# a-rtemis99/hpc_suffix_array

Measured on AMD Instinct MI355X. Metric: suffixes sorted/sec + ms/doubling-round, 1 GiB input at 1/2/4/8 MI355X, higher is better.
Workload: dtype u32

## Files before the change

hpc_suffix_array_amd/_native.py:

```python
from __future__ import annotations

import ctypes
import os
import subprocess

PKG_DIR = os.path.dirname(os.path.abspath(__file__))
LIB_PATH = os.path.join(PKG_DIR, "lib", "libsa_hip.so")
LIB_PATH = os.environ.get("SA_LIB_PATH", LIB_PATH)
CSRC = os.path.join(PKG_DIR, "csrc")

SA_MAX_ROUNDS = 64
KERNEL_KINDS = ["init", "hist_first", "hist_keys", "scan", "scatter_first", "scatter_keys",
                "heads", "heads_scan", "rerank", "seg_count", "seg_scan", "seg_write", "alphabet", "pack",
                "sort_u", "windows", "local_sort", "pivot_keys", "pivot_count", "pivot_write"]
SCHEDULE_PACKED = 0
SCHEDULE_REFERENCE = 1
ROUND1_AUTO = 0
ROUND1_LSD = 1
ROUND1_BUCKETED = 2
SA_K_COUNT = len(KERNEL_KINDS)
FIND_AUTO = 0
FIND_LANE = 1
FIND_WAVE = 2
FIND_LANE_MAX = 3584
FIND_MODES = {"auto": FIND_AUTO, "lane": FIND_LANE, "wave": FIND_WAVE}
BWT_STATS = 258
BWT_TILE = 4096

DROPIN_SYMBOLS = ["create_suffix_array", "destroy_suffix_array", "build_suffix_array",
                  "build_lcp_array", "find_longest_repeated_substring", "is_valid_suffix_array"]
EXT_SYMBOLS = ["sa_context_create", "sa_context_destroy", "sa_context_set_debug", "sa_workspace_bytes", "sa_build_device",
               "sa_build_ex", "sa_check_device", "sa_check", "sa_lcp_device", "sa_lcp", "sa_generate_text_device",
               "sa_alphabet_device", "sa_pack_keys_device", "sa_sort_pairs_device", "sa_scatter_u64_device",
               "sa_gather_u64_device", "sa_running_max_i64_device", "sa_inclusive_sum_i64_device",
               "sa_count_below_u64_device", "sa_select_u8_device",
               "sa_find_device", "sa_find", "sa_find_ex",
               "sa_match_device", "sa_matching_stats_device", "sa_match", "sa_matching_stats",
               "sa_bwt_device", "sa_bwt", "sa_inverse_device", "sa_inverse",
               "sa_dist_begin", "sa_dist_cuts", "sa_dist_plan_cuts", "sa_dist_reserve", "sa_dist_release", "sa_dist_round1", "sa_dist_req_count", "sa_dist_req_fill",
               "sa_dist_answer", "sa_dist_refine",
               "sa_last_error", "sa_host_syncs", "sa_device_count", "sa_version", "sa_struct_size"]


class SAError(RuntimeError):
    """A libsa_hip entry point returned an error code."""


DEBUG_FLAGS = {"no_cmp": 0x1, "no_pk8": 0x2, "no_pad": 0x4, "pad_overflow": 0x8, "no_fast32": 0x10,
               "no_pivot": 0x20, "perm_always": 0x40, "no_xq": 0x80, "xq_overflow": 0x100,
               "no_tied": 0x200, "no_key1_round": 0x400, "no_eonly": 0x800,
               "eonly": 0x1000, "fast32_small": 0x2000, "no_round2_fused": 0x4000}


def debug_bits(names) -> int:
    bits = 0
    for x in names or ():
        if x not in DEBUG_FLAGS:
            raise ValueError(f"unknown debug flag {x!r} (one of {sorted(DEBUG_FLAGS)})")
        bits |= DEBUG_FLAGS[x]
    return bits


class SaOpts(ctypes.Structure):
    _fields_ = [("profile", ctypes.c_int32), ("schedule", ctypes.c_int32), ("init_chars", ctypes.c_int32),
                ("radix", ctypes.c_int32), ("round1", ctypes.c_int32), ("debug", ctypes.c_uint32),
                ("span_extra", ctypes.c_int32), ("tune", ctypes.c_int32)]


class SaStats(ctypes.Structure):
    _fields_ = [
        ("rounds", ctypes.c_int32),
        ("n_kinds", ctypes.c_int32),
        ("total_ms", ctypes.c_double),
        ("h2d_ms", ctypes.c_double),
        ("d2h_ms", ctypes.c_double),
        ("round_ms", ctypes.c_double * SA_MAX_ROUNDS),
        ("distinct", ctypes.c_uint64 * SA_MAX_ROUNDS),
        ("passes", ctypes.c_int32 * SA_MAX_ROUNDS),
        ("sorted_n", ctypes.c_uint64 * SA_MAX_ROUNDS),
        ("prefix_len", ctypes.c_uint64 * SA_MAX_ROUNDS),
        ("schedule", ctypes.c_int32),
        ("init_chars", ctypes.c_int32),
        ("sigma", ctypes.c_int32),
        ("sparse_ranks", ctypes.c_int32),
        ("round1", ctypes.c_int32),
        ("largest_window", ctypes.c_int32),
        ("model_bytes", ctypes.c_uint64),
        ("kern_ms", ctypes.c_double * SA_K_COUNT),
        ("kern_launches", ctypes.c_uint64 * SA_K_COUNT),
        ("kern_bytes", ctypes.c_uint64 * SA_K_COUNT),
        ("round1_segments", ctypes.c_int32),
        ("round1_layout", ctypes.c_int32),
        ("round_bytes", ctypes.c_uint64 * SA_MAX_ROUNDS),
        ("round1_windows", ctypes.c_int32 * 4),
    ]

    def to_dict(self) -> dict:
        r = self.rounds
        return {
            "rounds": r,
            "total_ms": self.total_ms,
            "h2d_ms": self.h2d_ms,
            "d2h_ms": self.d2h_ms,
            "round_ms": list(self.round_ms[:r]),
# ... 187 lines not shown
```

hpc_suffix_array_amd/csrc/sa_bucket.h:

```cpp
#pragma once
#include "sa_kernels.h"

namespace sa {

#ifndef SA_BS_BLOCK
#define SA_BS_BLOCK 512
#endif
constexpr int kBsBlock = SA_BS_BLOCK;
#ifndef SA_BS_ITEMS
#define SA_BS_ITEMS 18
#endif
constexpr int kBsItems = SA_BS_ITEMS;
constexpr int kBsCap = kBsBlock * kBsItems;
constexpr uint32_t kWinStride = 1024;
#ifndef SA_BS_WPC
#define SA_BS_WPC 2
#endif
constexpr uint32_t kBsWpc = SA_BS_WPC;
#ifndef SA_BS_GRID
#define SA_BS_GRID (1u << 22)
#endif
constexpr uint32_t kBsGrid = SA_BS_GRID;
constexpr uint64_t kBucketMinN = 1ull << 20;
constexpr uint32_t kLoBits = 8;
constexpr uint32_t kLoRadix = 1u << kLoBits;

__device__ __forceinline__ uint32_t bucket_of(uint64_t key1, uint32_t rb, uint64_t cmul, uint32_t bsh) {
    return (uint32_t)(((key1 >> rb) * cmul) >> bsh);
}

__device__ __forceinline__ uint32_t bucket_dmin(uint32_t b, uint64_t cmul, uint32_t bsh) {
    const uint64_t d0 = ((uint64_t)b << bsh) / cmul;
    return (uint32_t)((((d0 * cmul) >> bsh) == b) ? d0 : d0 + 1);
}

struct SrcBucketKeys {
    const uint64_t* __restrict__ keys;
    const uint32_t* __restrict__ vals;
    uint32_t rb, bsh;
    uint64_t cmul;
    uint32_t bofs;
    __device__ __forceinline__ uint64_t key(uint64_t e) const { return keys[e]; }
    __device__ __forceinline__ uint32_t val(uint64_t e) const { return vals[e]; }
    static constexpr bool kPk8 = false;
    __device__ __forceinline__ uint32_t digit(uint64_t k, uint32_t shift, uint32_t mask) const {
        return ((bucket_of(k, rb, cmul, bsh) - bofs) >> shift) & mask;
    }
};

struct SrcPk8 {
    const uint64_t* __restrict__ items;
    __device__ __forceinline__ uint64_t key(uint64_t e) const { return items[e]; }
    __device__ __forceinline__ uint32_t val(uint64_t) const { return 0u; }
// ... 1363 lines not shown
        if constexpr (LSV & 1) {
            const uint32_t x = s_k[lo + t];
            v[t] = (uint32_t)t < cnt ? x : ~0u;
        } else {
            v[t] = (uint32_t)t < cnt ? s_k[lo + t] : ~0u;
        }
    }
    sort_net32<N>(v);
    uint32_t eqm = 0;
#pragma unroll
    for (int t = 0; t + 1 < N; ++t) eqm |= ((v[t] ^ v[t + 1]) <= kSlotMask ? 1u : 0u) << t;
    eqm &= (1u << (cnt - 1)) - 1u;
    if constexpr (LSV & 2) {
        if (eqm == 0u) {
            uint32_t xi[N];
#pragma unroll
            for (int t = 0; t < N; ++t) xi[t] = s_x[min(v[t] & kSlotMask, (uint32_t)kBsCap - 1u)];
#pragma unroll
            for (int t = 0; t < N; ++t)
                if ((uint32_t)t < cnt) s_k[lo + t] = xi[t];
            return false;
        }
    }
#pragma unroll
    for (int t = 0; t < N; ++t)
        if ((uint32_t)t < cnt) s_k[lo + t] = v[t];
    nu += (uint32_t)__popc(eqm | (eqm << 1));
    ng += (uint32_t)__popc(eqm & ~(eqm << 1));
    return eqm != 0u;
}

__device__ __forceinline__ void sort_sub_words_lds(uint32_t* __restrict__ s_k, uint32_t lo, uint32_t hi, uint32_t& nu,
                                                   uint32_t& ng) {
    for (uint32_t k = lo + 1; k < hi; ++k) {
        const uint32_t x = s_k[k];
        uint32_t y = k;
        while (y > lo && s_k[y - 1] > x) {
            s_k[y] = s_k[y - 1];
            --y;
        }
        s_k[y] = x;
    }
    uint32_t pr = ~0u, cur = s_k[lo] >> kSlotBits;
    for (uint32_t k = lo; k < hi; ++k) {
        const uint32_t nx = k + 1 < hi ? (s_k[k + 1] >> kSlotBits) : ~0u;
        const bool eqp = k > lo && pr == cur, eqn = k + 1 < hi && nx == cur;
        nu += (eqp || eqn) ? 1u : 0u;
        ng += (!eqp && eqn) ? 1u : 0u;
        pr = cur;
        cur = nx;
    }
}

template <int ITEMS>
__device__ __forceinline__ void load_items(const uint64_t* __restrict__ w_in, uint64_t a, uint32_t m,
                                           uint64_t (&x)[ITEMS]) {
    const uint32_t l0 = slot0<ITEMS>();
#pragma unroll
    for (int i = 0; i < ITEMS; ++i) {
        const uint32_t le = l0 + i * kWave;
        x[i] = w_in[a + (le < m ? le : m - 1)];
    }
}

struct XqWin {
    const uint32_t* __restrict__ hx = nullptr;
    const uint32_t* __restrict__ rows = nullptr;
};

__device__ __forceinline__ uint32_t xq_offset(const uint32_t* __restrict__ hx, uint32_t le) {
    uint32_t off = hx[0];
#pragma unroll
    for (int k = 1; k < (int)kXq; ++k) off = hx[kXq - 1 + k] <= le ? hx[k] : off;
    return off;
}

template <int ITEMS>
__device__ __forceinline__ void load_items_cr(const uint64_t* __restrict__ w_in, const uint32_t (&rv)[3],
                                              uint64_t (&x)[ITEMS]) {
    const uint32_t lane = lane_id();
#pragma unroll
    for (int i = 0; i < ITEMS; ++i) {
        const uint32_t base = (uint32_t)__builtin_amdgcn_readlane((int)rv[0], i);
        x[i] = (w_in + base)[lane];
    }
}

template <int ITEMS, int ROWS>
__device__ __forceinline__ void load_rows_xq(const uint32_t* __restrict__ rows, uint32_t (&rv)[3]) {
    const uint32_t lane = lane_id();
    const uint32_t w = (uint32_t)__builtin_amdgcn_readfirstlane((int)(threadIdx.x / kWave));
    const uint32_t r = w * ITEMS + (lane < (uint32_t)ITEMS ? lane : 0u);
#pragma unroll
    for (int t = 0; t < 3; ++t) rv[t] = rows[t * ROWS + r];
}

template <int ITEMS>
__device__ __forceinline__ void load_items_xq(const uint64_t* __restrict__ w_in, const uint32_t (&rv)[3], uint32_t m,
                                              uint64_t (&x)[ITEMS]) {
    const uint32_t l0 = slot0<ITEMS>();
    const uint32_t lane = lane_id();
    const uint32_t last = m - 1;
#pragma unroll
    for (int i = 0; i < ITEMS; ++i) {
        const uint32_t le = l0 + i * kWave;
        const uint32_t lc = le < m ? le : last;
        const uint32_t da = (uint32_t)__builtin_amdgcn_readlane((int)rv[0], i);
        const uint32_t db = (uint32_t)__builtin_amdgcn_readlane((int)rv[1], i);
        const uint32_t sp = (uint32_t)__builtin_amdgcn_readlane((int)rv[2], i);
        x[i] = w_in[(uint32_t)((lane < sp ? da : db) + lc)];
    }
}

template <bool CR>
__global__ __launch_bounds__(kBlock) void k_window_rows(const uint32_t* __restrict__ words, const uint4* __restrict__ hdr,
                                                        const uint32_t* __restrict__ hx, uint32_t nrows,
                                                        uint32_t* __restrict__ rows) {
    const uint32_t nh = words[kHdrWord];
    const uint32_t lane = lane_id();
    for (uint64_t q = (uint64_t)blockIdx.x * kWaves + wave_id(); q < nh; q += (uint64_t)gridDim.x * kWaves) {
        const uint32_t m = hdr[q].z;
        uint32_t hv[16];
#pragma unroll
        for (int k = 0; k < 16; ++k) hv[k] = hx[q * 16 + k];
        if constexpr (CR) {
            uint32_t st[kXq], cn[kXq], nfull = 0;
#pragma unroll
            for (int k = 0; k < (int)kXq; ++k) {
                const uint32_t p0 = k ? hv[kXq - 1 + k] : 0u, p1 = k + 1 < (int)kXq ? hv[kXq + k] : m;
                st[k] = hv[k] + p0;
                cn[k] = p1 - p0;
                nfull += cn[k] / kWave;
            }
            for (uint32_t r = lane; r < nrows; r += kWave) {
                uint32_t base = st[0], cnt = 0, rf = 0, rp = nfull;
#pragma unroll
                for (int k = 0; k < (int)kXq; ++k) {
                    const uint32_t nf = cn[k] / kWave, rem = cn[k] % kWave;
                    if (r >= rf && r < rf + nf) {
                        base = st[k] + kWave * (r - rf);
                        cnt = kWave;
                    }
                    if (rem && r == rp) {
                        base = st[k] + kWave * nf;
                        cnt = rem;
                    }
                    rf += nf;
                    rp += rem ? 1u : 0u;
                }
                uint32_t* const e = rows + q * 3 * nrows + r;
                e[0] = base;
                e[nrows] = cnt;
            }
            continue;
        }
        for (uint32_t r = lane; r < nrows; r += kWave) {
            const uint32_t lo = std::min(r * kWave, m - 1), hi = std::min(r * kWave + (kWave - 1), m - 1);
            uint32_t split = kWave;
#pragma unroll
            for (int k = kXq - 1; k >= 1; --k) {
                const uint32_t pk = hv[kXq - 1 + k];
                if (pk > lo && pk <= hi) split = pk - r * kWave;
            }
            uint32_t* const e = rows + q * 3 * nrows + r;
            e[0] = xq_offset(hv, lo);
            e[nrows] = xq_offset(hv, hi);
            e[2 * nrows] = split;
        }
    }
}

#ifndef SA_LS_WFULL
#define SA_LS_WFULL 1
#endif
#ifndef SA_LS_CLAIMS
#define SA_LS_CLAIMS 1
#endif
template <int BLOCK, int ITEMS, class Probe = NoProbe, bool XQ = false, int LSV = 0, bool CR = false>
__global__ __launch_bounds__(BLOCK, 4) void k_bucket_sort(const uint64_t* __restrict__ keys_in,
                                                       const uint4* __restrict__ hdr, uint32_t rb, uint32_t bits,
                                                       uint32_t ib, uint32_t* __restrict__ words,
                                                       uint64_t* __restrict__ keys_out, uint32_t* __restrict__ sa_out,
                                                       uint32_t* __restrict__ retry, SegOut so, XqWin xw = XqWin{}) {
    constexpr int WAVES = BLOCK / kWave;
    constexpr int CAP = BLOCK * ITEMS;
    static_assert(CAP <= (1 << kSlotBits), "load slots");
    __shared__ uint32_t s_lds[kSubBuckets / 2 + CAP + ((LSV & 1) ? kNet : 0) + CAP];
    uint32_t* const s_cnt = s_lds;
    uint32_t* const s_k = s_lds + kSubBuckets / 2;
    uint32_t* const s_x = s_k + CAP + ((LSV & 1) ? kNet : 0);
    __shared__ uint32_t s_tmp[WAVES];
    __shared__ uint32_t s_cm[WAVES];
    __shared__ uint32_t s_ug[WAVES];
    __shared__ uint32_t s_q[2];
    __shared__ unsigned long long s_tot[3];
    constexpr int WPT = kSubBuckets / 2 / BLOCK;
    static_assert(WPT * 2 == 4 && WPT * 2 * BLOCK == kSubBuckets, "four sub-buckets per thread");
    constexpr int ROWS = WAVES * ITEMS;

    const uint32_t wave = wave_id(), lane = lane_id();
    const uint32_t dg = threadIdx.x;
    const uint32_t nwin = words[kHdrWord];
    const uint32_t low_bits = bits - kSubBits;
    const uint32_t dsh = ib + low_bits;
    const uint32_t lmask = (1u << low_bits) - 1u;
    const uint64_t imask = (1ull << ib) - 1ull;
    auto end_of = [&](uint32_t sb) -> uint32_t { return ((s_cnt[sb >> 1] >> (16 * (sb & 1))) & 0xFFFFu) >> 2; };
    static_assert(4 * CAP < (1 << 16), "byte counts in 16-bit halves");
    auto cnt_word = [&](uint32_t y) -> uint32_t* {
        return reinterpret_cast<uint32_t*>(reinterpret_cast<char*>(s_cnt) + ((y << 1) & 0xFFCu));
    };
    auto half_inc = [](uint32_t y) -> uint32_t {
        uint32_t r;
        asm("v_lshlrev_b32_e64 %0, %1, 4" : "=v"(r) : "v"(y << 4));
        return r;
    };
    Probe probe;
    if (threadIdx.x == 0) {
        s_q[0] = atomicAdd(&words[kTicketWord], 1u);
        s_tot[0] = s_tot[1] = s_tot[2] = 0;
    }
    __syncthreads();
    uint32_t q = (uint32_t)__builtin_amdgcn_readfirstlane((int)s_q[0]);
    if (q >= nwin) return;
    uint4 h = hdr[q];
    uint64_t w[ITEMS];
    uint32_t rv[3] = {0u, 0u, 0u};
    if constexpr (XQ) {
        load_rows_xq<ITEMS, ROWS>(xw.rows + (uint64_t)q * 3 * ROWS, rv);
        if constexpr (CR) load_items_cr<ITEMS>(keys_in, rv, w);
        else load_items_xq<ITEMS>(keys_in, rv, h.z, w);
    } else {
        load_items<ITEMS>(keys_in, h.y, h.z, w);
    }
    uint32_t par = 0;
    for (;;) {
        probe.mark(-1);
        const uint32_t j = h.x, m = h.z;
        const uint64_t a = h.y;
        const uint64_t mn = (uint64_t)h.w << rb;
        if (threadIdx.x == 0) s_q[par ^ 1u] = atomicAdd(&words[kTicketWord], 1u);
        for (int i = threadIdx.x; i < kSubBuckets / 2; i += BLOCK) s_cnt[i] = 0;
        __syncthreads();
        const uint32_t qn = (uint32_t)__builtin_amdgcn_readfirstlane((int)s_q[par ^ 1u]);
        const bool more = qn < nwin;
        uint4 hn = make_uint4(0u, 0u, 1u, 0u);
        if (more) hn = hdr[qn];
        uint32_t rwn[3] = {0u, 0u, 0u};
        if constexpr (XQ) load_rows_xq<ITEMS, ROWS>(xw.rows + (uint64_t)(more ? qn : q) * 3 * ROWS, rwn);
        probe.mark(0);
        const uint32_t l0 = slot0<ITEMS>();
        const bool wfull = SA_LS_WFULL && (wave + 1) * (uint32_t)(kWave * ITEMS) <= m;
        bool sfull = wfull;
        if constexpr (XQ && CR)
            sfull = SA_LS_WFULL && __ballot(lane < (uint32_t)ITEMS && rv[1] == kWave) == (1ull << ITEMS) - 1ull;
        auto slot_ok = [&](int i) -> bool {
            if constexpr (XQ && CR) return lane < (uint32_t)__builtin_amdgcn_readlane((int)rv[1], i);
            else return l0 + i * kWave < m;
        };
        if (sfull) {
#pragma unroll
            for (int i = 0; i < ITEMS; ++i) {
                const uint32_t y = (uint32_t)(w[i] >> dsh);
                atomicAdd(cnt_word(y), half_inc(y));
            }
        } else {
#pragma unroll
            for (int i = 0; i < ITEMS; ++i) {
                if (slot_ok(i)) {
                    const uint32_t y = (uint32_t)(w[i] >> dsh);
                    atomicAdd(cnt_word(y), half_inc(y));
                }
            }
        }
        __syncthreads();
        probe.mark(1);
        uint32_t big = 0;
        {
            uint32_t c[2 * WPT], sum = 0, cm = 0;
#pragma unroll
            for (int x = 0; x < WPT; ++x) {
                const uint32_t pw = s_cnt[WPT * dg + x];
                c[2 * x] = pw & 0xFFFFu;
                c[2 * x + 1] = pw >> 16;
            }
#pragma unroll
            for (int x = 0; x < 2 * WPT; ++x) {
                sum += c[x];
                cm = c[x] > cm ? c[x] : cm;
            }
            const uint32_t inc = wave_inclusive_sum(sum);
#pragma unroll
            for (int o = kWave / 2; o > 0; o >>= 1) {
                const uint32_t y = __shfl_xor(cm, o, kWave);
                cm = y > cm ? y : cm;
            }
            if (lane == kWave - 1) s_tmp[wave] = inc;
            if (lane == 0) s_cm[wave] = cm;
            __syncthreads();
            uint32_t off = 0;
#pragma unroll
            for (int x = 0; x < WAVES; ++x) {
                off += (x < (int)wave) ? s_tmp[x] : 0u;
                big = s_cm[x] > big ? s_cm[x] : big;
            }
            uint32_t b = off + inc - sum;
#pragma unroll
            for (int x = 0; x < WPT; ++x) {
                const uint32_t b0 = b, b1 = b + c[2 * x];
                s_cnt[WPT * dg + x] = b0 | (b1 << 16);
                b = b1 + c[2 * x + 1];
            }
        }
        __syncthreads();
        probe.mark(2);
        if ((big >> 2) > kMaxSub) {
            if (threadIdx.x == 0) retry[atomicAdd(&words[kRetryWord], 1u)] = j;
            __builtin_amdgcn_sched_barrier(0);
            if constexpr (XQ && CR) load_items_cr<ITEMS>(keys_in, rwn, w);
            else if constexpr (XQ) load_items_xq<ITEMS>(keys_in, rwn, hn.z, w);
            else load_items<ITEMS>(keys_in, hn.y, hn.z, w);
            __syncthreads();
        } else {
            auto scatter1 = [&](int i, uint32_t le) {
                const uint32_t y = (uint32_t)(w[i] >> dsh);
                const uint32_t old = atomicAdd(cnt_word(y), half_inc(y));
                const uint32_t at = __builtin_amdgcn_ubfe(old, y << 4, 16u);
                *reinterpret_cast<uint32_t*>(reinterpret_cast<char*>(s_k) + at) =
                    (((uint32_t)(w[i] >> ib) & lmask) << kSlotBits) | le;
                s_x[le] = (uint32_t)(w[i] & imask);
            };
            if (sfull) {
#pragma unroll
                for (int g = 0; g < ITEMS; g += SA_LS_CLAIMS) {
                    uint32_t y[SA_LS_CLAIMS], old[SA_LS_CLAIMS];
#pragma unroll
                    for (int t = 0; t < SA_LS_CLAIMS; ++t) {
                        y[t] = (uint32_t)(w[g + t] >> dsh);
                        old[t] = atomicAdd(cnt_word(y[t]), half_inc(y[t]));
                    }
#pragma unroll
                    for (int t = 0; t < SA_LS_CLAIMS; ++t) {
                        const int i = g + t;
                        const uint32_t le = l0 + i * kWave;
                        const uint32_t at = __builtin_amdgcn_ubfe(old[t], y[t] << 4, 16u);
                        *reinterpret_cast<uint32_t*>(reinterpret_cast<char*>(s_k) + at) =
                            (((uint32_t)(w[i] >> ib) & lmask) << kSlotBits) | le;
                        s_x[le] = (uint32_t)(w[i] & imask);
                    }
                }
            } else {
#pragma unroll
                for (int i = 0; i < ITEMS; ++i) {
                    const uint32_t le = l0 + i * kWave;
                    if (slot_ok(i)) scatter1(i, le);
                }
            }
            __builtin_amdgcn_sched_barrier(0);
            if constexpr (XQ && CR) load_items_cr<ITEMS>(keys_in, rwn, w);
            else if constexpr (XQ) load_items_xq<ITEMS>(keys_in, rwn, hn.z, w);
            else load_items<ITEMS>(keys_in, hn.y, hn.z, w);
            __syncthreads();
            probe.mark(3);
            uint32_t nu = 0, ng = 0;
            uint32_t umask = 0;
            const uint32_t sb0 = 2 * WPT * dg;
            uint32_t order = 0;
            {
                uint32_t o[4];
#pragma unroll
                for (int k = 0; k < 4; ++k) {
                    const uint32_t sb = sb0 + k;
                    o[k] = ((end_of(sb) - (sb ? end_of(sb - 1) : 0u)) << 2) | (uint32_t)k;
                }
                sort_net32<4>(o);
#pragma unroll
                for (int k = 0; k < 4; ++k) order |= (o[3 - k] & 3u) << (2 * k);
            }
#pragma unroll 1
            for (uint32_t i = 0; i < 4; ++i) {
                const uint32_t sb = sb0 + ((order >> (2 * i)) & 3u);
                const uint32_t lo = sb ? end_of(sb - 1) : 0u, hi = end_of(sb), cnt = hi - lo;
                const bool wide4 = __ballot(cnt > 4u) != 0ull, wide8 = __ballot(cnt > 8u) != 0ull,
                           wide12 = __ballot(cnt > 12u) != 0ull;
                if (cnt == 0) continue;
                const uint32_t nu0 = nu;
                constexpr int LW = LSV & 1;
                bool grp;
                if ((LSV & 2) && !so.samples) {
                    if (!wide4) grp = sort_sub_words<4, LSV>(s_k, s_x, lo, cnt, nu, ng);
                    else if (!wide8) grp = sort_sub_words<8, LSV>(s_k, s_x, lo, cnt, nu, ng);
                    else if (!wide12) grp = sort_sub_words<12, LSV>(s_k, s_x, lo, cnt, nu, ng);
                    else if (cnt <= (uint32_t)kNet) grp = sort_sub_words<kNet, LSV>(s_k, s_x, lo, cnt, nu, ng);
                    else {
                        sort_sub_words_lds(s_k, lo, hi, nu, ng);
                        grp = true;
                    }
                } else {
                    if (!wide4) sort_sub_words<4, LW>(s_k, s_x, lo, cnt, nu, ng);
                    else if (!wide8) sort_sub_words<8, LW>(s_k, s_x, lo, cnt, nu, ng);
                    else if (!wide12) sort_sub_words<12, LW>(s_k, s_x, lo, cnt, nu, ng);
                    else if (cnt <= (uint32_t)kNet) sort_sub_words<kNet, LW>(s_k, s_x, lo, cnt, nu, ng);
                    else sort_sub_words_lds(s_k, lo, hi, nu, ng);
                    grp = nu != nu0;
                }
                if (grp) umask |= 1u << (sb - sb0);
                if (so.samples)
                    for_each_sample(a, lo, hi, so.ksh, [&](uint32_t q) {
                        keys_out[(a + q) >> so.ksh] = mn + (((uint64_t)sb << low_bits) | (s_k[q] >> kSlotBits));
                    });
            }
            probe.mark(4);
            uint32_t bu, bg, tu_w, tg_w;
            {
                const uint32_t iug = wave_inclusive_sum(nu | (ng << 16));
                if (lane == kWave - 1) s_ug[wave] = iug;
                __syncthreads();
                uint32_t oug = 0, tug = 0;
#pragma unroll
                for (int x = 0; x < WAVES; ++x) {
                    const uint32_t xug = s_ug[x];
                    oug += (x < (int)wave) ? xug : 0u;
                    tug += xug;
                }
                tu_w = tug & 0xFFFFu;
                tg_w = tug >> 16;
                bu = (oug & 0xFFFFu) + (iug & 0xFFFFu) - nu;
                bg = (oug >> 16) + (iug >> 16) - ng;
            }
            const bool idx_back = (LSV & 2) && !so.samples;
            if (so.rank && threadIdx.x == 0) {
                so.cnt_u[j] = tu_w;
                so.cnt_g[j] = tg_w;
                s_tot[0] += m - tu_w + tg_w;
                s_tot[1] += tu_w;
                s_tot[2] += tg_w;
            }
            if (umask && (so.rank || idx_back)) {
                uint32_t ku = bu, kg = bg;
                for (uint32_t um = umask; um; um &= um - 1u) {
                    const uint32_t sb = sb0 + (uint32_t)__builtin_ctz(um);
                    const uint32_t lo = sb ? end_of(sb - 1) : 0u, hi = end_of(sb);
                    uint32_t head = lo, pr = ~0u;
                    for (uint32_t k = lo; k < hi; ++k) {
                        const uint32_t v = s_k[k], r = v >> kSlotBits;
                        const uint32_t nx = k + 1 < hi ? (s_k[k + 1] >> kSlotBits) : ~0u;
                        const bool eqp = k > lo && pr == r, eqn = k + 1 < hi && nx == r;
                        const uint32_t xi = s_x[v & kSlotMask];
                        if (idx_back) s_k[k] = xi;
                        if (!eqp) head = k;
                        if (!eqp && eqn) ++kg;
                        if (so.rank && (eqp || eqn)) {
                            const uint32_t rv = (uint32_t)(so.rank_off + a + head + 1u);
                            if (so.tmp_rank) so.tmp_rank[a + ku] = rv;
                            else so.rank[xi] = rv;
                            atomicOr(&so.member[xi >> 5], 1u << (xi & 31));
                            so.tmp_pos[a + ku] = (uint32_t)(a + k);
                            so.tmp_idx[a + ku] = xi;
                            so.tmp_g[a + ku] = kg - 1u;
                            ++ku;
                        }
                        pr = r;
                    }
                }
            }
            probe.mark(5);
            if (idx_back) {
                __syncthreads();
                if (wfull) {
#pragma unroll 2
                    for (int i = 0; i < ITEMS; ++i) {
                        const uint32_t le = l0 + i * kWave;
                        sa_out[a + le] = s_k[le];
                    }
                } else {
#pragma unroll 2
                    for (int i = 0; i < ITEMS; ++i) {
                        const uint32_t le = l0 + i * kWave;
                        if (le < m) sa_out[a + le] = s_k[le];
                    }
                }
            } else if (wfull) {
#pragma unroll 2
                for (int i = 0; i < ITEMS; ++i) {
                    const uint32_t le = l0 + i * kWave;
                    sa_out[a + le] = s_x[s_k[le] & kSlotMask];
                }
            } else {
#pragma unroll 2
                for (int i = 0; i < ITEMS; ++i) {
                    const uint32_t le = l0 + i * kWave;
                    if (le < m) sa_out[a + le] = s_x[s_k[le] & kSlotMask];
                }
            }
            __syncthreads();
            probe.mark(6);
        }
        if (!more) break;
        q = qn;
        h = hn;
        if constexpr (XQ && CR) {
            rv[0] = rwn[0];
            rv[1] = rwn[1];
        }
        par ^= 1u;
    }
    probe.flush(words);
    __syncthreads();
    flush_totals(words, s_tot[0], s_tot[1], s_tot[2]);
}

template <int BLOCK, int ITEMS>
__global__ __launch_bounds__(BLOCK) void k_bucket_sort_lsd(const uint64_t* __restrict__ keys_in, BucketRel br,
                                                           const uint32_t* __restrict__ ws,
                                                           const uint32_t* __restrict__ skew,
                                                           uint32_t* __restrict__ words, uint32_t ib,
                                                           uint64_t* __restrict__ keys_out,
                                                           uint32_t* __restrict__ sa_out, SegOut so) {
    constexpr int WAVES = BLOCK / kWave;
    constexpr int CAP = BLOCK * ITEMS;
    constexpr int WT = kWave * ITEMS;
    static_assert(BLOCK >= kRadix, "one thread per digit");
    static_assert(CAP <= 65535, "16-bit LDS offsets");
    __shared__ uint64_t s_w[CAP];
    __shared__ uint16_t s_wcnt[WAVES][kRadix];
    __shared__ uint16_t s_start[kRadix];
    __shared__ uint32_t s_tmp[kWaves];
    __shared__ uint64_t s_red[2][WAVES];
    __shared__ uint32_t s_bk[2][32];

    const uint32_t wave = wave_id(), lane = lane_id();
    const uint32_t dg = threadIdx.x;
    uint32_t* err = words + 6;
    const uint32_t nskew = words[10];
    static_assert(WAVES * ITEMS * 8 <= WAVES * kRadix * 2, "per-row segment values fit in s_wcnt");
    uint64_t th = 0, tu = 0, tg = 0;
    for (uint32_t q = blockIdx.x; q < nskew; q += gridDim.x) {
        const uint32_t j = skew[q];
        const uint64_t a = ws[j];
        const uint32_t m = (uint32_t)(ws[j + 1] - a);
        uint64_t w[ITEMS];
        uint64_t mn;
        uint32_t bits;
        if (!load_window<BLOCK, ITEMS>(keys_in, br, j, a, m, ib, w, mn, bits, s_red, s_bk, err)) {
            __syncthreads();
            continue;
        }
        const uint32_t passes = (bits + 7) / 8;
        for (uint32_t p = 0; p < passes; ++p) {
            const uint32_t sh = ib + 8 * p;
            for (int i = threadIdx.x; i < WAVES * kRadix; i += BLOCK) (&s_wcnt[0][0])[i] = 0;
            __syncthreads();
            uint32_t r[ITEMS];
            uint16_t* wc = s_wcnt[wave];
#pragma unroll
            for (int i = 0; i < ITEMS; ++i) {
// ... 71 lines not shown
```

hpc_suffix_array_amd/csrc/sa_round1.h:

```cpp
#pragma once

#ifndef SA_HIST_WPC
#define SA_HIST_WPC 64
#endif
#ifndef SA_REC_STRIPED
#define SA_REC_STRIPED 1
#endif
#ifndef SA_BB_EXTRA
#define SA_BB_EXTRA 0
#endif
#ifndef SA_ITEMS_A
#define SA_ITEMS_A 12
#endif
#ifndef SA_TEXT_BLOCK
#define SA_TEXT_BLOCK 512
#endif
#ifndef SA_LIST_BLOCK
#define SA_LIST_BLOCK 1024
#endif


#ifndef SA_SEG_BLOCK
#define SA_SEG_BLOCK 1024
#endif
// ... 480 lines not shown
        hipLaunchKernelGGL(k_window_list, dim3(g2), dim3(kBlock), 0, s, (const uint32_t*)ws, nw, list, c->words);
    }
    tm.end();
    add_bytes(st, SA_K_WINDOWS, 8 * nw);
    SA_HIP(hipGetLastError());
    SA_HIP(hipMemcpyAsync(c->host_words, c->words, 48, hipMemcpyDeviceToHost, s));
    uint32_t* skew = list + nw;
    uint32_t* cnt_u = skew + nw;
    uint32_t* cnt_g = cnt_u + nw + 1;
    uint32_t* const rank_arr = br_.rank ? br_.rank : c->rank;
    uint32_t* const member = br_.member ? br_.member : c->member;
    SA_HIP(hipEventRecord(c->ev[kSyncEv], s));
    SA_HIP(hipMemsetAsync(cnt_u, 0, (2 * nw + 2) * 4, s));
    SA_HIP(hipMemsetAsync(member, 0, (n + 31) / 32 * 4, s));
    SA_HIP(host_sync_event(c->ev[kSyncEv]));
    if (c->host_words[4]) return set_err(SA_E_INTERNAL, "radix look-back did not complete");
    if (padded && c->host_words[11]) {
        SA_TRACE("  bucketed round 1: padded segment overflow, again with exact digit totals");
        const int rc = round1_bucketed(c, d_text, n, d_sa, bp, br_, s, tm, st, done, fused, seg, ksh, false, allow_xq,
                                       round2);
        if (st) st->round1_segments = 2;
        return rc;
    }
    if (xq && c->host_words[9]) {
        SA_TRACE("  bucketed round 1: second-pass queue overflow, again with one region");
        return round1_bucketed(c, d_text, n, d_sa, bp, br_, s, tm, st, done, fused, seg, ksh, allow_pad, false,
                               round2);
    }
    if (st) st->largest_window = (int32_t)std::min<uint32_t>(c->host_words[5], INT32_MAX);
    if (c->host_words[5] > (uint32_t)kBsCap) {
        SA_TRACE("  bucketed round 1: window of %u > %d suffixes, full sort instead", c->host_words[5], kBsCap);
        return SA_OK;
    }
    BucketRel br{cnt_g + nw + 1, c->segw + kBstartOff, c->segw + kBstartOff + kBstartWords, bp.bs.rb};
    br.bits1 = bits1;
    SegOut so{rank_arr, member, br_.sa_off, c->u_pos[1], c->u_idx[1], c->u_g[1], cnt_u, cnt_g, kKeySample};
    so.tmp_rank = br_.prefix ? br_.tmp_rank : nullptr;
    so.samples = (SA_LAZY_SAMPLES && !br_.always_u && !(c->dbg & SA_DEBUG_NO_KEY1_ROUND)) ? 0u : 1u;
    uint32_t* const retry = cnt_g + 2 * nw + 2;
    BucketRel br_measured = br;
    br_measured.bits1 = 0;
    uint4* const hdr = reinterpret_cast<uint4*>(((uintptr_t)(retry + nw + 4) + 15) & ~(uintptr_t)15);
    uint32_t* const hx = xq ? reinterpret_cast<uint32_t*>(hdr + nw + 1) : nullptr;
    constexpr uint32_t kBsRows = (kBsBlock / kWave) * kBsItems;
    uint32_t* const xrows = xq ? hx + 16 * (nw + 1) : nullptr;
    const uint64_t* const wide_in = xq ? c->keys[1] : c->keys_u;
    auto local_sort = [&](const SegOut& o) {
        const uint32_t g = std::max<uint32_t>(1, std::min(c->host_words[7], kBsGrid));
        static_assert(kRetryWord == kUsFlagWord + 1, "one memset clears words[12..15]");
        (void)hipMemsetAsync(c->words + kUsFlagWord, 0, 16, s);
        if (fast32) {
            const uint32_t gs = (uint32_t)std::max<uint64_t>(1, std::min<uint64_t>((nw + kBlock - 1) / kBlock, 1024));
            const bool cr = xq && !(((uint32_t)c->tune >> 29) & 1u);
            hipLaunchKernelGGL(k_window_split, dim3(gs), dim3(kBlock), 0, s, (const uint32_t*)list, (const uint32_t*)ws,
                               br, c->words, hdr, retry, 1u, (const uint32_t*)xq_pc, (const uint32_t*)xq_pn, nb_tab, hx,
                               cr ? kBsRows : 0u);
            if (xq) {
                if (cr)
                    hipLaunchKernelGGL(k_window_rows<true>, dim3(2048), dim3(kBlock), 0, s, (const uint32_t*)c->words,
                                       (const uint4*)hdr, (const uint32_t*)hx, kBsRows, xrows);
                else
                    hipLaunchKernelGGL(k_window_rows<false>, dim3(2048), dim3(kBlock), 0, s, (const uint32_t*)c->words,
                                       (const uint4*)hdr, (const uint32_t*)hx, kBsRows, xrows);
                XqWin xw;
                xw.hx = hx;
                xw.rows = xrows;
#define SA_LS_XQ(V, CR)                                                                                          \
    hipLaunchKernelGGL((k_bucket_sort<kBsBlock, kBsItems, NoProbe, true, V, CR>), dim3(kBsWpc * (uint32_t)c->cus), \
                       dim3(kBsBlock), 0, s, (const uint64_t*)c->keys_u, (const uint4*)hdr, bp.bs.rb, br.bits1,  \
                       bp.ib, c->words, c->keys[0], d_sa, retry, o, xw)
                switch (ls_variant(c) | (cr ? 4 : 0)) {
                case 1: SA_LS_XQ(1, false); break;
                case 2: SA_LS_XQ(2, false); break;
                case 3: SA_LS_XQ(3, false); break;
                case 4: SA_LS_XQ(0, true); break;
                case 5: SA_LS_XQ(1, true); break;
                case 6: SA_LS_XQ(2, true); break;
                case 7: SA_LS_XQ(3, true); break;
                default: SA_LS_XQ(0, false); break;
                }
#undef SA_LS_XQ
                hipLaunchKernelGGL(k_window_gather, dim3(1024), dim3(kBlock), 0, s, (const uint32_t*)retry,
                                   (const uint32_t*)c->words, (const uint32_t*)ws, (const uint32_t*)br.wb,
                                   (const uint32_t*)xq_pc, (const uint32_t*)xq_pn, nb_tab, (const uint64_t*)c->keys_u,
                                   c->keys[1]);
            } else {
#define SA_LS(V)                                                                                                 \
    hipLaunchKernelGGL((k_bucket_sort<kBsBlock, kBsItems, NoProbe, false, V>), dim3(kBsWpc * (uint32_t)c->cus),  \
                       dim3(kBsBlock), 0, s, (const uint64_t*)c->keys_u, (const uint4*)hdr, bp.bs.rb, br.bits1,  \
                       bp.ib, c->words, c->keys[0], d_sa, retry, o)
                switch (ls_variant(c)) {
                case 1: SA_LS(1); break;
                case 2: SA_LS(2); break;
                case 3: SA_LS(3); break;
                default: SA_LS(0); break;
                }
#undef SA_LS
            }
        } else {
            hipLaunchKernelGGL((k_bucket_sort_wide<kBsBlock, kBsItems>), dim3(g), dim3(kBsBlock), 0, s,
                               (const uint64_t*)c->keys_u, br, (const uint32_t*)ws, (const uint32_t*)list, c->words,
                               bp.ib, c->keys[0], d_sa, skew, o, br.bits1 ? retry : (uint32_t*)nullptr, 7u);
        }
        if (br.bits1)
            hipLaunchKernelGGL((k_bucket_sort_wide<kBsBlock, kBsItems>), dim3(std::min<uint32_t>(g, 1024)),
                               dim3(kBsBlock), 0, s, wide_in, br_measured, (const uint32_t*)ws,
                               (const uint32_t*)retry, c->words, bp.ib, c->keys[0], d_sa, skew, o, (uint32_t*)nullptr,
                               (uint32_t)kRetryWord);
        const uint32_t gl = std::min<uint32_t>(g, 1024);
        hipLaunchKernelGGL((k_bucket_sort_lsd<kBsBlock, kBsItems>), dim3(gl), dim3(kBsBlock), 0, s,
                           wide_in, br, (const uint32_t*)ws, (const uint32_t*)skew, c->words, bp.ib,
                           c->keys[0], d_sa, o);
    };
    tm.begin(SA_K_LOCAL_SORT);
    local_sort(so);
    tm.end();
    add_bytes(st, SA_K_LOCAL_SORT, 12 * m + (so.samples ? (m >> kKeySample) * 8 : 0));
    SA_HIP(hipGetLastError());
    auto gather_u = [&]() {
        const uint32_t wb = (uint32_t)((nw + 1 + kWsBlock - 1) / kWsBlock);
        uint32_t* part = c->hist;
        hipLaunchKernelGGL(k_wscan_reduce, dim3(wb), dim3(kBlock), 0, s, (const uint32_t*)cnt_u, (const uint32_t*)cnt_g,
                           nw, part);
        hipLaunchKernelGGL(k_wscan_top, dim3(1), dim3(kBlock), 0, s, part, wb);
        hipLaunchKernelGGL(k_wscan_apply, dim3(wb), dim3(kBlock), 0, s, cnt_u, cnt_g, nw, (const uint32_t*)part);
        const uint32_t g = (uint32_t)std::max<uint64_t>(1, std::min<uint64_t>((c->host_words[7] + kWaves - 1) / kWaves, 4096));
        RankMap rm;
        if (br_.prefix) {
            const uint64_t nwb = (n + 31) / 32;
            const uint32_t pb = (uint32_t)((nwb + kPcBlock - 1) / kPcBlock);
            uint32_t* ppart = br_.prefix + nwb + 1;
            hipLaunchKernelGGL(k_popc_reduce, dim3(pb), dim3(kBlock), 0, s, (const uint32_t*)member, nwb, ppart);
            hipLaunchKernelGGL(k_popc_top, dim3(1), dim3(kPcTop), 0, s, ppart, pb);
            hipLaunchKernelGGL(k_popc_apply, dim3(pb), dim3(kBlock), 0, s, (const uint32_t*)member, nwb,
                               (const uint32_t*)ppart, br_.prefix);
            rm = RankMap{member, br_.prefix};
        }
        hipLaunchKernelGGL(k_u_gather, dim3(g), dim3(kBlock), 0, s, (const uint32_t*)list, (const uint32_t*)c->words,
                           (const uint32_t*)ws, (const uint32_t*)cnt_u, (const uint32_t*)cnt_g, so, c->u_pos[0],
                           c->u_idx[0], c->u_g[0], rm);
    };
    const bool try_r2 = round2 && so.rank && !br_.always_u && !so.tmp_rank && br_.sa_off == 0 &&
                        !(c->dbg & (SA_DEBUG_NO_KEY1_ROUND | SA_DEBUG_NO_ROUND2_FUSED)) && key1_bits(bp.bs) <= 64;
// ... 70 lines not shown
```

include/sa_hip.h:

```cpp
#ifndef SA_HIP_H
#define SA_HIP_H

#include <stdint.h>

#ifdef __cplusplus
extern "C" {
#endif

#define SA_OK 0
#define SA_E_INVALID (-1)
#define SA_E_NOMEM (-2)
#define SA_E_HIP (-3)
#define SA_E_INTERNAL (-4)

#define SA_MAX_ROUNDS 64

enum sa_kernel_kind {
    SA_K_INIT = 0,
    SA_K_HIST_FIRST = 1,
    SA_K_HIST_KEYS = 2,
    SA_K_SCAN = 3,
    SA_K_SCATTER_FIRST = 4,
    SA_K_SCATTER_KEYS = 5,
    SA_K_HEADS = 6,
    SA_K_HEADS_SCAN = 7,
    SA_K_RERANK = 8,
    SA_K_SEG_COUNT = 9,
    SA_K_SEG_SCAN = 10,
    SA_K_SEG_WRITE = 11,
    SA_K_ALPHABET = 12,
    SA_K_PACK = 13,
    SA_K_SORT_U = 14,
    SA_K_WINDOWS = 15,
    SA_K_LOCAL_SORT = 16,
    SA_K_PIVOT_KEYS = 17,
    SA_K_PIVOT_COUNT = 18,
    SA_K_PIVOT_WRITE = 19,
    SA_K_COUNT = 20
};

#define SA_ROUND1_AUTO 0
#define SA_ROUND1_LSD 1
#define SA_ROUND1_BUCKETED 2
#define SA_ROUND1_PIVOT 3

#define SA_SCHEDULE_PACKED 0
#define SA_SCHEDULE_REFERENCE 1

#define SA_DEBUG_NO_CMP 0x1u
#define SA_DEBUG_NO_PK8 0x2u
#define SA_DEBUG_NO_PAD 0x4u
#define SA_DEBUG_PAD_OVERFLOW 0x8u
#define SA_DEBUG_NO_FAST32 0x10u
#define SA_DEBUG_NO_PIVOT 0x20u
#define SA_DEBUG_PERM_ALWAYS 0x40u
#define SA_DEBUG_NO_XQ 0x80u
#define SA_DEBUG_XQ_OVERFLOW 0x100u
#define SA_DEBUG_NO_KEY1_ROUND 0x400u
#define SA_DEBUG_NO_TIED 0x200u
#define SA_DEBUG_NO_EONLY 0x800u
#define SA_DEBUG_EONLY 0x1000u
#define SA_DEBUG_FAST32_SMALL 0x2000u
#define SA_DEBUG_NO_ROUND2_FUSED 0x4000u

typedef struct {
    int32_t profile;
    int32_t schedule;
    int32_t init_chars;
    int32_t radix;
    int32_t round1;
    uint32_t debug;
    int32_t span_extra;
    int32_t tune;
} sa_opts;

typedef struct {
    int32_t rounds;
    int32_t n_kinds;
    double total_ms;
    double h2d_ms, d2h_ms;
    double round_ms[SA_MAX_ROUNDS];
    uint64_t distinct[SA_MAX_ROUNDS];
    int32_t passes[SA_MAX_ROUNDS];
    uint64_t sorted_n[SA_MAX_ROUNDS];
    uint64_t prefix_len[SA_MAX_ROUNDS];
    int32_t schedule;
    int32_t init_chars;
    int32_t sigma;
    int32_t sparse_ranks;
    int32_t round1;
    int32_t largest_window;
    uint64_t model_bytes;
    double kern_ms[SA_K_COUNT];
    uint64_t kern_launches[SA_K_COUNT];
    uint64_t kern_bytes[SA_K_COUNT];
    int32_t round1_segments;
    int32_t round1_layout;
    uint64_t round_bytes[SA_MAX_ROUNDS];
    int32_t round1_windows[4];
} sa_stats;

typedef struct sa_context sa_context;

int sa_context_create(int device, uint64_t max_n, sa_context** out);
int sa_context_set_debug(sa_context* ctx, const sa_opts* opts);
void sa_context_destroy(sa_context* ctx);
uint64_t sa_workspace_bytes(uint64_t max_n);

int sa_build_device(sa_context* ctx, const uint8_t* d_text, uint64_t n, uint32_t* d_sa,
                    void* stream, const sa_opts* opts, sa_stats* stats);

int sa_build_ex(const uint8_t* text, uint64_t n, void* sa_out, int sa_width,
                const sa_opts* opts, sa_stats* stats);

int sa_check_device(sa_context* ctx, const uint8_t* d_text, uint64_t n, const uint32_t* d_sa,
                    void* stream);
// ... 118 lines not shown
```

Measured before the change: 105.6 billion.

## Hoist local-sort rank capture into count pass and stagger next-window prefetch

The persistent bucket-sort kernel now records each item's within-sub-bucket rank (byte ranks from the count atomics) during the histogram pass, so the scatter phase places keys with no second round of LDS atomics. It claims the next window's ticket one iteration ahead, so the per-window ticket, counter-clear and barrier preamble goes away. The next window's key loads are split into chunks issued at several points through the sort, spreading memory latency instead of one bulk load. The cost is more registers held across the loop (keys, packed ranks, bucket bounds), which can lower occupancy. A debug flag that launches a single workgroup is also added.

```diff
diff --git a/hpc_suffix_array_amd/_native.py b/hpc_suffix_array_amd/_native.py
--- a/hpc_suffix_array_amd/_native.py
+++ b/hpc_suffix_array_amd/_native.py
@@ -49,7 +49,8 @@
 DEBUG_FLAGS = {"no_cmp": 0x1, "no_pk8": 0x2, "no_pad": 0x4, "pad_overflow": 0x8, "no_fast32": 0x10,
                "no_pivot": 0x20, "perm_always": 0x40, "no_xq": 0x80, "xq_overflow": 0x100,
                "no_tied": 0x200, "no_key1_round": 0x400, "no_eonly": 0x800,
-               "eonly": 0x1000, "fast32_small": 0x2000, "no_round2_fused": 0x4000}
+               "eonly": 0x1000, "fast32_small": 0x2000, "no_round2_fused": 0x4000,
+               "ls_one_wg": 0x8000}
 
 
 def debug_bits(names) -> int:
diff --git a/hpc_suffix_array_amd/csrc/sa_bucket.h b/hpc_suffix_array_amd/csrc/sa_bucket.h
--- a/hpc_suffix_array_amd/csrc/sa_bucket.h
+++ b/hpc_suffix_array_amd/csrc/sa_bucket.h
@@ -1,4 +1,6 @@
 #pragma once
+#include <type_traits>
+
 #include "sa_kernels.h"
 
 namespace sa {
@@ -1468,12 +1470,12 @@
     }
 }
 
-template <int ITEMS>
+template <int ITEMS, int I0 = 0, int I1 = ITEMS>
 __device__ __forceinline__ void load_items(const uint64_t* __restrict__ w_in, uint64_t a, uint32_t m,
                                            uint64_t (&x)[ITEMS]) {
     const uint32_t l0 = slot0<ITEMS>();
 #pragma unroll
-    for (int i = 0; i < ITEMS; ++i) {
+    for (int i = I0; i < I1; ++i) {
         const uint32_t le = l0 + i * kWave;
         x[i] = w_in[a + (le < m ? le : m - 1)];
     }
@@ -1491,12 +1493,12 @@
     return off;
 }
 
-template <int ITEMS>
+template <int ITEMS, int I0 = 0, int I1 = ITEMS>
 __device__ __forceinline__ void load_items_cr(const uint64_t* __restrict__ w_in, const uint32_t (&rv)[3],
                                               uint64_t (&x)[ITEMS]) {
     const uint32_t lane = lane_id();
 #pragma unroll
-    for (int i = 0; i < ITEMS; ++i) {
+    for (int i = I0; i < I1; ++i) {
         const uint32_t base = (uint32_t)__builtin_amdgcn_readlane((int)rv[0], i);
         x[i] = (w_in + base)[lane];
     }
@@ -1511,14 +1513,14 @@
     for (int t = 0; t < 3; ++t) rv[t] = rows[t * ROWS + r];
 }
 
-template <int ITEMS>
+template <int ITEMS, int I0 = 0, int I1 = ITEMS>
 __device__ __forceinline__ void load_items_xq(const uint64_t* __restrict__ w_in, const uint32_t (&rv)[3], uint32_t m,
                                               uint64_t (&x)[ITEMS]) {
     const uint32_t l0 = slot0<ITEMS>();
     const uint32_t lane = lane_id();
     const uint32_t last = m - 1;
 #pragma unroll
-    for (int i = 0; i < ITEMS; ++i) {
+    for (int i = I0; i < I1; ++i) {
         const uint32_t le = l0 + i * kWave;
         const uint32_t lc = le < m ? le : last;
         const uint32_t da = (uint32_t)__builtin_amdgcn_readlane((int)rv[0], i);
@@ -1592,6 +1594,27 @@
 #ifndef SA_LS_CLAIMS
 #define SA_LS_CLAIMS 1
 #endif
+#ifndef SA_LS_HRANK
+#define SA_LS_HRANK 1
+#endif
+#ifndef SA_LS_HRANK_PF
+#define SA_LS_HRANK_PF 3
+#endif
+#if SA_LS_HRANK_PF == 0
+#define SA_LS_PF_TABLE {0, 0, 18, 18, 18}
+#elif SA_LS_HRANK_PF == 1
+#define SA_LS_PF_TABLE {18, 18, 18, 18, 18}
+#elif SA_LS_HRANK_PF == 3
+#define SA_LS_PF_TABLE {6, 6, 12, 18, 18}
+#elif SA_LS_HRANK_PF == 5
+#define SA_LS_PF_TABLE {0, 0, 6, 12, 18}
+#elif SA_LS_HRANK_PF == 6
+#define SA_LS_PF_TABLE {3, 6, 9, 15, 18}
+#endif
+constexpr int kLsPfHr[5] = SA_LS_PF_TABLE;
+constexpr int kLsPfOld[5] = {0, 0, 18, 18, 18};
+template <int P>
+using pf_point = std::integral_constant<int, P>;
 template <int BLOCK, int ITEMS, class Probe = NoProbe, bool XQ = false, int LSV = 0, bool CR = false>
 __global__ __launch_bounds__(BLOCK, 4) void k_bucket_sort(const uint64_t* __restrict__ keys_in,
                                                        const uint4* __restrict__ hdr, uint32_t rb, uint32_t bits,
@@ -1631,11 +1654,16 @@
         asm("v_lshlrev_b32_e64 %0, %1, 4" : "=v"(r) : "v"(y << 4));
         return r;
     };
+    constexpr bool HR = SA_LS_HRANK != 0;
+    typedef uint16_t __attribute__((may_alias)) half_t;
     Probe probe;
     if (threadIdx.x == 0) {
         s_q[0] = atomicAdd(&words[kTicketWord], 1u);
+        if constexpr (HR) s_q[1] = atomicAdd(&words[kTicketWord], 1u);
         s_tot[0] = s_tot[1] = s_tot[2] = 0;
     }
+    if constexpr (HR)
+        for (int i = threadIdx.x; i < kSubBuckets / 2; i += BLOCK) s_cnt[i] = 0;
     __syncthreads();
     uint32_t q = (uint32_t)__builtin_amdgcn_readfirstlane((int)s_q[0]);
     if (q >= nwin) return;
@@ -1649,21 +1677,31 @@
     } else {
         load_items<ITEMS>(keys_in, h.y, h.z, w);
     }
+    uint32_t qn = 0;
+    bool more = false;
+    uint4 hn = make_uint4(0u, 0u, 1u, 0u);
+    uint32_t rwn[3] = {0u, 0u, 0u};
+    auto next_window = [&](uint32_t ticket, uint32_t cur, uint32_t& qx, bool& mx, uint4& hx,
+                           uint32_t (&rx)[3]) __attribute__((always_inline)) {
+        qx = (uint32_t)__builtin_amdgcn_readfirstlane((int)ticket);
+        mx = qx < nwin;
+        hx = make_uint4(0u, 0u, 1u, 0u);
+        if (mx) hx = hdr[qx];
+        if constexpr (XQ) load_rows_xq<ITEMS, ROWS>(xw.rows + (uint64_t)(mx ? qx : cur) * 3 * ROWS, rx);
+    };
+    if constexpr (HR) next_window(s_q[1], q, qn, more, hn, rwn);
     uint32_t par = 0;
     for (;;) {
         probe.mark(-1);
         const uint32_t j = h.x, m = h.z;
         const uint64_t a = h.y;
         const uint64_t mn = (uint64_t)h.w << rb;
-        if (threadIdx.x == 0) s_q[par ^ 1u] = atomicAdd(&words[kTicketWord], 1u);
-        for (int i = threadIdx.x; i < kSubBuckets / 2; i += BLOCK) s_cnt[i] = 0;
-        __syncthreads();
-        const uint32_t qn = (uint32_t)__builtin_amdgcn_readfirstlane((int)s_q[par ^ 1u]);
-        const bool more = qn < nwin;
-        uint4 hn = make_uint4(0u, 0u, 1u, 0u);
-        if (more) hn = hdr[qn];
-        uint32_t rwn[3] = {0u, 0u, 0u};
-        if constexpr (XQ) load_rows_xq<ITEMS, ROWS>(xw.rows + (uint64_t)(more ? qn : q) * 3 * ROWS, rwn);
+        if constexpr (!HR) {
+            if (threadIdx.x == 0) s_q[par ^ 1u] = atomicAdd(&words[kTicketWord], 1u);
+            for (int i = threadIdx.x; i < kSubBuckets / 2; i += BLOCK) s_cnt[i] = 0;
+            __syncthreads();
+            next_window(s_q[par ^ 1u], q, qn, more, hn, rwn);
+        }
         probe.mark(0);
         const uint32_t l0 = slot0<ITEMS>();
         const bool wfull = SA_LS_WFULL && (wave + 1) * (uint32_t)(kWave * ITEMS) <= m;
@@ -1674,7 +1712,49 @@
             if constexpr (XQ && CR) return lane < (uint32_t)__builtin_amdgcn_readlane((int)rv[1], i);
             else return l0 + i * kWave < m;
         };
-        if (sfull) {
+        static_assert(ITEMS == 18, "SA_LS_PF_TABLE");
+        auto prefetch_at = [&](auto pc, auto rest) __attribute__((always_inline)) {
+            constexpr int P = decltype(pc)::value;
+            constexpr int A = P ? (HR ? kLsPfHr[P - 1] : kLsPfOld[P - 1]) : 0;
+            constexpr int B = decltype(rest)::value ? ITEMS : (HR ? kLsPfHr[P] : kLsPfOld[P]);
+            if constexpr (A < B) {
+                __builtin_amdgcn_sched_barrier(0);
+                if constexpr (XQ && CR) load_items_cr<ITEMS, A, B>(keys_in, rwn, w);
+                else if constexpr (XQ) load_items_xq<ITEMS, A, B>(keys_in, rwn, hn.z, w);
+                else load_items<ITEMS, A, B>(keys_in, hn.y, hn.z, w);
+            }
+        };
+        constexpr std::false_type part{};
+        constexpr std::true_type rest{};
+        constexpr int RKW = (ITEMS + 3) / 4;
+        uint32_t kk[HR ? ITEMS : 1], rk[HR ? RKW : 1];
+        uint32_t tk = 0;
+        static_assert(4 * kMaxSub <= 256, "byte ranks in 8 bits");
+        if constexpr (HR) {
+#pragma unroll
+            for (int r = 0; r < RKW; ++r) rk[r] = 0;
+            auto count1 = [&](int i, uint32_t le) {
+                const uint32_t k = (uint32_t)(w[i] >> ib);
+                const uint32_t y = k >> low_bits;
+                const uint32_t old = atomicAdd(cnt_word(y), half_inc(y));
+                s_x[le] = (uint32_t)(w[i] & imask);
+                kk[i] = k;
+                rk[i / 4] |= __builtin_amdgcn_ubfe(old, y << 4, 8u) << (8 * (i % 4));
+            };
+            if (sfull) {
+#pragma unroll
+                for (int i = 0; i < ITEMS; ++i) count1(i, l0 + i * kWave);
+            } else {
+#pragma unroll
+                for (int i = 0; i < ITEMS; ++i) {
+                    kk[i] = 0;
+                    if (slot_ok(i)) count1(i, l0 + i * kWave);
+                }
+            }
+            __builtin_amdgcn_sched_barrier(0);
+            if (threadIdx.x == 0) tk = atomicAdd(&words[kTicketWord], 1u);
+            prefetch_at(pf_point<0>{}, part);
+        } else if (sfull) {
 #pragma unroll
             for (int i = 0; i < ITEMS; ++i) {
                 const uint32_t y = (uint32_t)(w[i] >> dsh);
@@ -1692,6 +1772,7 @@
         __syncthreads();
         probe.mark(1);
         uint32_t big = 0;
+        uint32_t bw[2 * WPT + 1];
         {
             uint32_t c[2 * WPT], sum = 0, cm = 0;
 #pragma unroll
@@ -1726,18 +1807,36 @@
                 const uint32_t b0 = b, b1 = b + c[2 * x];
                 s_cnt[WPT * dg + x] = b0 | (b1 << 16);
                 b = b1 + c[2 * x + 1];
-            }
-        }
+                bw[2 * x] = b0 >> 2;
+                bw[2 * x + 1] = b1 >> 2;
+            }
+            bw[2 * WPT] = b >> 2;
+            if constexpr (HR)
+                if (threadIdx.x == 0) s_q[0] = tk;
+        }
+        prefetch_at(pf_point<1>{}, part);
         __syncthreads();
         probe.mark(2);
+        uint32_t qnn = 0;
+        bool moren = false;
+        uint4 hnn = make_uint4(0u, 0u, 1u, 0u);
+        uint32_t rwnn[3] = {0u, 0u, 0u};
         if ((big >> 2) > kMaxSub) {
             if (threadIdx.x == 0) retry[atomicAdd(&words[kRetryWord], 1u)] = j;
-            __builtin_amdgcn_sched_barrier(0);
-            if constexpr (XQ && CR) load_items_cr<ITEMS>(keys_in, rwn, w);
-            else if constexpr (XQ) load_items_xq<ITEMS>(keys_in, rwn, hn.z, w);
-            else load_items<ITEMS>(keys_in, hn.y, hn.z, w);
+            if constexpr (HR) {
+#pragma unroll
+                for (int x = 0; x < WPT; ++x) s_cnt[WPT * dg + x] = 0;
+            }
+            prefetch_at(pf_point<2>{}, rest);
             __syncthreads();
+            if constexpr (HR) next_window(s_q[0], q, qnn, moren, hnn, rwnn);
         } else {
+            auto place1 = [&](int i, uint32_t le) {
+                const uint32_t k = kk[HR ? i : 0];
+                const uint32_t st = reinterpret_cast<const half_t*>(s_cnt)[(k >> low_bits) & (uint32_t)(kSubBuckets - 1)];
+                const uint32_t at = st + __builtin_amdgcn_ubfe(rk[HR ? i / 4 : 0], 8u * (i % 4), 8u);
+                *reinterpret_cast<uint32_t*>(reinterpret_cast<char*>(s_k) + at) = ((k & lmask) << kSlotBits) | le;
+            };
             auto scatter1 = [&](int i, uint32_t le) {
                 const uint32_t y = (uint32_t)(w[i] >> dsh);
                 const uint32_t old = atomicAdd(cnt_word(y), half_inc(y));
@@ -1746,7 +1845,18 @@
                     (((uint32_t)(w[i] >> ib) & lmask) << kSlotBits) | le;
                 s_x[le] = (uint32_t)(w[i] & imask);
             };
-            if (sfull) {
+            (void)place1;
+            (void)scatter1;
+            if constexpr (HR) {
+                if (sfull) {
+#pragma unroll
+                    for (int i = 0; i < ITEMS; ++i) place1(i, l0 + i * kWave);
+                } else {
+#pragma unroll
+                    for (int i = 0; i < ITEMS; ++i)
+                        if (slot_ok(i)) place1(i, l0 + i * kWave);
+                }
+            } else if (sfull) {
 #pragma unroll
                 for (int g = 0; g < ITEMS; g += SA_LS_CLAIMS) {
                     uint32_t y[SA_LS_CLAIMS], old[SA_LS_CLAIMS];
@@ -1772,22 +1882,34 @@
                     if (slot_ok(i)) scatter1(i, le);
                 }
             }
-            __builtin_amdgcn_sched_barrier(0);
-            if constexpr (XQ && CR) load_items_cr<ITEMS>(keys_in, rwn, w);
-            else if constexpr (XQ) load_items_xq<ITEMS>(keys_in, rwn, hn.z, w);
-            else load_items<ITEMS>(keys_in, hn.y, hn.z, w);
+            prefetch_at(pf_point<2>{}, part);
             __syncthreads();
+            if constexpr (HR) next_window(s_q[0], q, qnn, moren, hnn, rwnn);
             probe.mark(3);
             uint32_t nu = 0, ng = 0;
             uint32_t umask = 0;
             const uint32_t sb0 = 2 * WPT * dg;
+            auto sub_range = [&](uint32_t k, uint32_t& lo, uint32_t& hi) __attribute__((always_inline)) {
+                if constexpr (HR) {
+                    static_assert(WPT == 2, "four sub-buckets per thread");
+                    lo = bw[3], hi = bw[4];
+                    if (k == 0) lo = bw[0], hi = bw[1];
+                    if (k == 1) lo = bw[1], hi = bw[2];
+                    if (k == 2) lo = bw[2], hi = bw[3];
+                } else {
+                    const uint32_t sb = sb0 + k;
+                    lo = sb ? end_of(sb - 1) : 0u;
+                    hi = end_of(sb);
+                }
+            };
             uint32_t order = 0;
             {
                 uint32_t o[4];
 #pragma unroll
                 for (int k = 0; k < 4; ++k) {
-                    const uint32_t sb = sb0 + k;
-                    o[k] = ((end_of(sb) - (sb ? end_of(sb - 1) : 0u)) << 2) | (uint32_t)k;
+                    uint32_t lo, hi;
+                    sub_range((uint32_t)k, lo, hi);
+                    o[k] = ((hi - lo) << 2) | (uint32_t)k;
                 }
                 sort_net32<4>(o);
 #pragma unroll
@@ -1796,7 +1918,9 @@
 #pragma unroll 1
             for (uint32_t i = 0; i < 4; ++i) {
                 const uint32_t sb = sb0 + ((order >> (2 * i)) & 3u);
-                const uint32_t lo = sb ? end_of(sb - 1) : 0u, hi = end_of(sb), cnt = hi - lo;
+                uint32_t lo, hi;
+                sub_range(sb - sb0, lo, hi);
+                const uint32_t cnt = hi - lo;
                 const bool wide4 = __ballot(cnt > 4u) != 0ull, wide8 = __ballot(cnt > 8u) != 0ull,
                            wide12 = __ballot(cnt > 12u) != 0ull;
                 if (cnt == 0) continue;
@@ -1826,6 +1950,7 @@
                         keys_out[(a + q) >> so.ksh] = mn + (((uint64_t)sb << low_bits) | (s_k[q] >> kSlotBits));
                     });
             }
+            prefetch_at(pf_point<3>{}, part);
             probe.mark(4);
             uint32_t bu, bg, tu_w, tg_w;
             {
@@ -1844,6 +1969,10 @@
                 bu = (oug & 0xFFFFu) + (iug & 0xFFFFu) - nu;
                 bg = (oug >> 16) + (iug >> 16) - ng;
             }
+            if constexpr (HR) {
+#pragma unroll
+                for (int x = 0; x < WPT; ++x) s_cnt[WPT * dg + x] = 0;
+            }
             const bool idx_back = (LSV & 2) && !so.samples;
             if (so.rank && threadIdx.x == 0) {
                 so.cnt_u[j] = tu_w;
@@ -1855,8 +1984,8 @@
             if (umask && (so.rank || idx_back)) {
                 uint32_t ku = bu, kg = bg;
                 for (uint32_t um = umask; um; um &= um - 1u) {
-                    const uint32_t sb = sb0 + (uint32_t)__builtin_ctz(um);
-                    const uint32_t lo = sb ? end_of(sb - 1) : 0u, hi = end_of(sb);
+                    uint32_t lo, hi;
+                    sub_range((uint32_t)__builtin_ctz(um), lo, hi);
                     uint32_t head = lo, pr = ~0u;
                     for (uint32_t k = lo; k < hi; ++k) {
                         const uint32_t v = s_k[k], r = v >> kSlotBits;
@@ -1880,6 +2009,7 @@
                     }
                 }
             }
+            prefetch_at(pf_point<4>{}, part);
             probe.mark(5);
             if (idx_back) {
                 __syncthreads();
@@ -1918,6 +2048,13 @@
         if constexpr (XQ && CR) {
             rv[0] = rwn[0];
             rv[1] = rwn[1];
+        }
+        if constexpr (HR) {
+            qn = qnn;
+            more = moren;
+            hn = hnn;
+#pragma unroll
+            for (int t = 0; t < 3; ++t) rwn[t] = rwnn[t];
         }
         par ^= 1u;
     }
diff --git a/hpc_suffix_array_amd/csrc/sa_round1.h b/hpc_suffix_array_amd/csrc/sa_round1.h
--- a/hpc_suffix_array_amd/csrc/sa_round1.h
+++ b/hpc_suffix_array_amd/csrc/sa_round1.h
@@ -556,6 +556,7 @@
         if (fast32) {
             const uint32_t gs = (uint32_t)std::max<uint64_t>(1, std::min<uint64_t>((nw + kBlock - 1) / kBlock, 1024));
             const bool cr = xq && !(((uint32_t)c->tune >> 29) & 1u);
+            const uint32_t ls_grid = (c->dbg & SA_DEBUG_LS_ONE_WG) ? 1u : kBsWpc * (uint32_t)c->cus;
             hipLaunchKernelGGL(k_window_split, dim3(gs), dim3(kBlock), 0, s, (const uint32_t*)list, (const uint32_t*)ws,
                                br, c->words, hdr, retry, 1u, (const uint32_t*)xq_pc, (const uint32_t*)xq_pn, nb_tab, hx,
                                cr ? kBsRows : 0u);
@@ -570,9 +571,9 @@
                 xw.hx = hx;
                 xw.rows = xrows;
 #define SA_LS_XQ(V, CR)                                                                                          \
-    hipLaunchKernelGGL((k_bucket_sort<kBsBlock, kBsItems, NoProbe, true, V, CR>), dim3(kBsWpc * (uint32_t)c->cus), \
-                       dim3(kBsBlock), 0, s, (const uint64_t*)c->keys_u, (const uint4*)hdr, bp.bs.rb, br.bits1,  \
-                       bp.ib, c->words, c->keys[0], d_sa, retry, o, xw)
+    hipLaunchKernelGGL((k_bucket_sort<kBsBlock, kBsItems, NoProbe, true, V, CR>), dim3(ls_grid), dim3(kBsBlock), 0, \
+                       s, (const uint64_t*)c->keys_u, (const uint4*)hdr, bp.bs.rb, br.bits1, bp.ib, c->words,      \
+                       c->keys[0], d_sa, retry, o, xw)
                 switch (ls_variant(c) | (cr ? 4 : 0)) {
                 case 1: SA_LS_XQ(1, false); break;
                 case 2: SA_LS_XQ(2, false); break;
@@ -590,9 +591,9 @@
                                    c->keys[1]);
             } else {
 #define SA_LS(V)                                                                                                 \
-    hipLaunchKernelGGL((k_bucket_sort<kBsBlock, kBsItems, NoProbe, false, V>), dim3(kBsWpc * (uint32_t)c->cus),  \
-                       dim3(kBsBlock), 0, s, (const uint64_t*)c->keys_u, (const uint4*)hdr, bp.bs.rb, br.bits1,  \
-                       bp.ib, c->words, c->keys[0], d_sa, retry, o)
+    hipLaunchKernelGGL((k_bucket_sort<kBsBlock, kBsItems, NoProbe, false, V>), dim3(ls_grid), dim3(kBsBlock), 0, \
+                       s, (const uint64_t*)c->keys_u, (const uint4*)hdr, bp.bs.rb, br.bits1, bp.ib, c->words,   \
+                       c->keys[0], d_sa, retry, o)
                 switch (ls_variant(c)) {
                 case 1: SA_LS(1); break;
                 case 2: SA_LS(2); break;
diff --git a/include/sa_hip.h b/include/sa_hip.h
--- a/include/sa_hip.h
+++ b/include/sa_hip.h
@@ -62,6 +62,7 @@
 #define SA_DEBUG_EONLY 0x1000u
 #define SA_DEBUG_FAST32_SMALL 0x2000u
 #define SA_DEBUG_NO_ROUND2_FUSED 0x4000u
+#define SA_DEBUG_LS_ONE_WG 0x8000u
 
 typedef struct {
     int32_t profile;
```

Measured after the change: 108.7 billion, median of 6. 1.03x the previous value.
